# vlongle/pixie

Measured on AMD Instinct MI355X. Metric: voxels/s (128^3 U-Net fwd) + MPM particle-steps/s, higher is better.
Workload: dtype f32 (operands split fp16 hi+lo, 3 f16 MFMAs/product, fp32 accumulate); 1 GPU; 128^3x64 feature grid -> SegmentationUNet+RegressionUNet forward (+argmax/one-hot combine), 1 scene per GPU per step; grid=128, feature_channels=64, parallelism=scene-parallel x1, executor=c+hip_graph

## Files before the change

pixie_amd/csrc/conv3d_f16x3.hip:

```cpp
#include <hip/hip_runtime.h>

#include <cstdlib>
#include <map>
#include <string>
#include <type_traits>

#include "../../include/pixie_hip.h"
#include "common.h"
#include "conv_plan.h"

namespace pixie {

typedef float f32x16 __attribute__((ext_vector_type(16)));
typedef _Float16 f16x8 __attribute__((ext_vector_type(8)));

constexpr int kW16HeaderU4 = 4;

struct Conv16Args {
    const float* in0; const float* in1;
    int c0, cin;
    int ID, IH, IW;
    int LD, LH, LW;
    int ups;
    int stride;
    int OD, OH, OW;
    const float* pro_a; const float* pro_b; const float* gamma; const float* beta;
    int act;
    const uint4* w16;
    const float* wf;
    const float* bias;
    int cout, coutp;
    const float* residual; float* out;
    const unsigned* amax0; const unsigned* amax1;
    float in_bound;
    int TX, TY, TZ, lTX, lTY;
    int tiles_x, tiles_y, tiles_z, n_tiles;
    int HX, HY, HZ, HYX, CS;
    unsigned mHX, mHYX;
    float* stats; unsigned* out_amax;
    float* partial; int chunks_per_slice;
    int epi_lds;
    const float* sk_in0; const float* sk_in1;
    int sk_c0, sk_cin;
    const uint4* sk_w16; const float* sk_bias;
    const unsigned* sk_amax0; const unsigned* sk_amax1;
};

__device__ __forceinline__ int fast_div16(int n, int d, unsigned magic) {
    return (d == 1) ? n : (int)__umulhi((unsigned)n, magic);
}
__device__ __forceinline__ float act16(float t, int act) {
    if (act == 1) return t > 0.0f ? t : 0.02f * t;
    if (act == 2) return t / (1.0f + __expf(-t));
    return t;
}
__device__ __forceinline__ int scale_exponent(float bound) {
    const unsigned bits = __float_as_uint(bound);
    const int eb = (int)((bits >> 23) & 0xffu) - 127;
    if (!(bound > 0.0f) || eb > 100) return 0;
    int e = 14 - eb;
    return e > 100 ? 100 : (e < -100 ? -100 : e);
}
__device__ __forceinline__ float pow2i(int e) { return __uint_as_float((unsigned)(e + 127) << 23); }

template <int KS, int MB, int NB, bool EX = false, bool SP = false>
__device__ __forceinline__ void conv3d_f16x3_body(const Conv16Args& A) {
    static_assert(!SP || (KS == 3 && NB == 4 && !EX), "sub-pixel path: 3^3, two x parities x two voxel blocks per wave");
    extern __shared__ uint4 smem16[];
    constexpr int PAD = (KS == 3) ? 1 : 0;
    constexpr int NW = 4, NT = 64 * NW;
    const int bufsz = 4 * A.CS;

    const int tid = threadIdx.x;
    const int lane = tid & 63;
    const int wave = tid >> 6;
    const int kh = lane >> 5;
    const int l31 = lane & 31;

    int t = blockIdx.x;
    {
        const int per = (A.n_tiles + 7) >> 3;
        const int cand = (t & 7) * per + (t >> 3);
        if ((A.n_tiles & 7) == 0) t = cand;
    }
    int par = 0;
    if constexpr (SP) { par = t & 3; t >>= 2; }
    const int py = par & 1, pz = par >> 1;
    const int tx = t % A.tiles_x; t /= A.tiles_x;
    const int ty = t % A.tiles_y;
    const int tz = t / A.tiles_y;
    const int ox0 = tx * A.TX, oy0 = ty * A.TY, oz0 = tz * A.TZ;
    const int cout0 = blockIdx.y * (MB * 32);
    const int lx0 = SP ? ox0 - 1 : ox0 * A.stride - PAD;
    const int ly0 = SP ? oy0 - 1 + py : oy0 * A.stride - PAD;
    const int lz0 = SP ? oz0 - 1 + pz : oz0 * A.stride - PAD;
    const size_t ISP = (size_t)A.ID * A.IH * A.IW;
    const size_t OSP = (size_t)A.OD * A.OH * A.OW;

    int voff[NB];
    int ovox[NB];
    bool valid[NB];
#pragma unroll
    for (int nb = 0; nb < NB; ++nb) {
        if constexpr (SP) {
            const int px = nb >> 1;
            const int j = (wave * 2 + (nb & 1)) * 32 + l31;
            int x = j & (A.TX - 1);
            int y = (j >> A.lTX) & (A.TY - 1);
            int z = j >> (A.lTX + A.lTY);
            const int gx = 2 * (ox0 + x) + px, gy = 2 * (oy0 + y) + py, gz = 2 * (oz0 + z) + pz;
            const bool v = (z < A.TZ) && (gx < A.OW) && (gy < A.OH) && (gz < A.OD);
            if (!v) { x = 0; y = 0; z = 0; }
            voff[nb] = (z * A.HY + y) * A.HX + x + px + kh * A.CS;
            ovox[nb] = v ? (gz * A.OH + gy) * A.OW + gx : 0;
            valid[nb] = v;
            continue;
        }
        const int j = (wave * NB + nb) * 32 + l31;
        int x = j & (A.TX - 1);
        int y = (j >> A.lTX) & (A.TY - 1);
        int z = j >> (A.lTX + A.lTY);
        const bool v = (z < A.TZ) && (ox0 + x < A.OW) && (oy0 + y < A.OH) && (oz0 + z < A.OD);
        if (!v) { x = 0; y = 0; z = 0; }
        voff[nb] = ((z * A.HY + y) * A.HX + x) * A.stride + kh * A.CS;
        ovox[nb] = ((oz0 + z) * A.OH + (oy0 + y)) * A.OW + ox0 + x;
        valid[nb] = v;
    }

    float bound = A.in_bound;
    if (A.amax0) {
        bound = __uint_as_float(*A.amax0);
        if (A.amax1) bound = fmaxf(bound, __uint_as_float(*A.amax1));
    }
    const int ex = EX ? 0 : scale_exponent(bound);
    const float sx = pow2i(ex);

    f32x16 acc[MB][NB];
#pragma unroll
    for (int mb = 0; mb < MB; ++mb)
#pragma unroll
        for (int nb = 0; nb < NB; ++nb)
#pragma unroll
            for (int r = 0; r < 16; ++r) acc[mb][nb][r] = 0.0f;

    const int KG = A.cin >> 3;
    const size_t tap_stride = (size_t)KG * A.coutp;
    const size_t plane = (size_t)(SP ? 64 : KS * KS * KS) * tap_stride;
    const uint4* wHi = A.w16 + kW16HeaderU4 + (size_t)kh * A.coutp + cout0 + l31 + (size_t)(par * 16) * tap_stride;
    const uint4* wLo = wHi + plane;
    const float* wF = A.wf + (size_t)kh * A.coutp + cout0 + l31;
// ... 220 lines not shown
                        bl[s] = __builtin_bit_cast(f16x8, ldsLo[voff[px * 2 + s] + rowoff + ex]);
                    }
#pragma unroll
                    for (int mb = 0; mb < MB; ++mb)
#pragma unroll
                        for (int s = 0; s < 2; ++s)
                            acc[mb][px * 2 + s] = __builtin_amdgcn_mfma_f32_32x32x16_f16(al[mb], bh[s], acc[mb][px * 2 + s], 0, 0, 0);
#pragma unroll
                    for (int mb = 0; mb < MB; ++mb)
#pragma unroll
                        for (int s = 0; s < 2; ++s)
                            acc[mb][px * 2 + s] = __builtin_amdgcn_mfma_f32_32x32x16_f16(ah[mb], bl[s], acc[mb][px * 2 + s], 0, 0, 0);
#pragma unroll
                    for (int mb = 0; mb < MB; ++mb)
#pragma unroll
                        for (int s = 0; s < 2; ++s)
                            acc[mb][px * 2 + s] = __builtin_amdgcn_mfma_f32_32x32x16_f16(ah[mb], bh[s], acc[mb][px * 2 + s], 0, 0, 0);
#pragma unroll
                    for (int mb = 0; mb < MB; ++mb) { ah[mb] = ahn[mb]; al[mb] = aln[mb]; }
                }
            }
            __builtin_amdgcn_s_setprio(0);
            return;
        }
        f16x8 ah[MB], al[MB];
#pragma unroll
        for (int mb = 0; mb < MB; ++mb) {
            ah[mb] = __builtin_bit_cast(f16x8, wh[mb * 32]);
            al[mb] = __builtin_bit_cast(f16x8, wl[mb * 32]);
        }
#pragma unroll 1
        for (int zy = 0; zy < KS * KS; ++zy) {
            const int dz = zy / KS, dy = zy - dz * KS;
            const int rowoff = (dz * A.HY + dy) * A.HX;
#pragma unroll
            for (int dx = 0; dx < KS; ++dx) {
                const int tap = zy * KS + dx;
                const int nxt = (tap + 1 < TAPS) ? tap + 1 : tap;
                f16x8 ahn[MB], aln[MB];
#pragma unroll
                for (int mb = 0; mb < MB; ++mb) {
                    ahn[mb] = __builtin_bit_cast(f16x8, wh[(size_t)nxt * tap_stride + mb * 32]);
                    aln[mb] = __builtin_bit_cast(f16x8, wl[(size_t)nxt * tap_stride + mb * 32]);
                }
                __builtin_amdgcn_sched_barrier(0);
                f16x8 bh[NB], bl[NB];
#pragma unroll
                for (int nb = 0; nb < NB; ++nb) {
                    bh[nb] = __builtin_bit_cast(f16x8, ldsHi[voff[nb] + rowoff + dx]);
                    bl[nb] = __builtin_bit_cast(f16x8, ldsLo[voff[nb] + rowoff + dx]);
                }
#pragma unroll
                for (int mb = 0; mb < MB; ++mb)
#pragma unroll
                    for (int nb = 0; nb < NB; ++nb)
                        acc[mb][nb] = __builtin_amdgcn_mfma_f32_32x32x16_f16(al[mb], bh[nb], acc[mb][nb], 0, 0, 0);
#pragma unroll
                for (int mb = 0; mb < MB; ++mb)
#pragma unroll
                    for (int nb = 0; nb < NB; ++nb)
                        acc[mb][nb] = __builtin_amdgcn_mfma_f32_32x32x16_f16(ah[mb], bl[nb], acc[mb][nb], 0, 0, 0);
#pragma unroll
                for (int mb = 0; mb < MB; ++mb)
#pragma unroll
                    for (int nb = 0; nb < NB; ++nb)
                        acc[mb][nb] = __builtin_amdgcn_mfma_f32_32x32x16_f16(ah[mb], bh[nb], acc[mb][nb], 0, 0, 0);
#pragma unroll
                for (int mb = 0; mb < MB; ++mb) { ah[mb] = ahn[mb]; al[mb] = aln[mb]; }
            }
        }
        __builtin_amdgcn_s_setprio(0);
    };

    float inv2 = 0.0f;
    {
        const int c_begin = A.partial ? (int)blockIdx.z * A.chunks_per_slice * 16 : 0;
        const int c_end = A.partial ? min(A.cin, c_begin + A.chunks_per_slice * 16) : A.cin;
        for (int c_base = c_begin; c_base < c_end; c_base += 16) {
            __syncthreads();
            stage_chunk(c_base, smem16, tid, NT);
            __syncthreads();
            mfma_chunk(c_base, smem16);
        }
        if (!EX && !SP && A.sk_w16) {
            float sb = __uint_as_float(*A.sk_amax0);
            if (A.sk_amax1) sb = fmaxf(sb, __uint_as_float(*A.sk_amax1));
            const int ex2 = scale_exponent(sb);
            const float sx2 = pow2i(ex2);
            const float inv_main = __uint_as_float(A.w16[0].x) * pow2i(-ex);
            inv2 = __uint_as_float(A.sk_w16[0].x) * pow2i(-ex2);
            const float ratio = inv_main / inv2;
#pragma unroll
            for (int mb = 0; mb < MB; ++mb)
#pragma unroll
                for (int nb = 0; nb < NB; ++nb)
#pragma unroll
                    for (int r = 0; r < 16; ++r) acc[mb][nb][r] *= ratio;
            const int KG2 = A.sk_cin >> 3;
            const uint4* w2Hi = A.sk_w16 + kW16HeaderU4 + (size_t)kh * A.coutp + cout0 + l31;
            const uint4* w2Lo = w2Hi + (size_t)KG2 * A.coutp;
            const int centre = (KS == 3) ? (A.HY + 1) * A.HX + 1 : 0;
            const int tvox = A.TX * A.TY * A.TZ;
            for (int c2 = 0; c2 < A.sk_cin; c2 += 16) {
                f16x8 ah[MB], al[MB];
#pragma unroll
                for (int mb = 0; mb < MB; ++mb) {
                    ah[mb] = __builtin_bit_cast(f16x8, w2Hi[(size_t)(c2 >> 3) * A.coutp + mb * 32]);
                    al[mb] = __builtin_bit_cast(f16x8, w2Lo[(size_t)(c2 >> 3) * A.coutp + mb * 32]);
                }
                __syncthreads();
                uint4* bHi = smem16;
                uint4* bLo = smem16 + 2 * A.CS;
                for (int j = tid; j < tvox; j += NT) {
                    const int x = j & (A.TX - 1), y = (j >> A.lTX) & (A.TY - 1), z = j >> (A.lTX + A.lTY);
                    const bool okv = (ox0 + x < A.OW) && (oy0 + y < A.OH) && (oz0 + z < A.OD);
                    const size_t sidx = okv ? ((size_t)(oz0 + z) * A.IH + (oy0 + y)) * A.IW + ox0 + x : 0;
                    float val[16];
#pragma unroll
                    for (int q = 0; q < 16; ++q) {
                        const int cg = c2 + q;
                        const float* src = (cg < A.sk_c0) ? (A.sk_in0 + (size_t)cg * ISP) : (A.sk_in1 + (size_t)(cg - A.sk_c0) * ISP);
                        val[q] = src[sidx];
                    }
                    f16x8 vh[2], vl[2];
#pragma unroll
                    for (int q = 0; q < 16; ++q) {
                        const float sc = okv ? val[q] * sx2 : 0.0f;
                        const _Float16 hq = (_Float16)sc;
                        vh[q >> 3][q & 7] = hq;
                        vl[q >> 3][q & 7] = (_Float16)(sc - (float)hq);
                    }
                    const int slot = (z * A.HY + y) * A.HX + x + centre;
                    bHi[slot] = __builtin_bit_cast(uint4, vh[0]);
                    bHi[A.CS + slot] = __builtin_bit_cast(uint4, vh[1]);
                    bLo[slot] = __builtin_bit_cast(uint4, vl[0]);
                    bLo[A.CS + slot] = __builtin_bit_cast(uint4, vl[1]);
                }
                __syncthreads();
                f16x8 bh[NB], bl[NB];
#pragma unroll
                for (int nb = 0; nb < NB; ++nb) {
                    bh[nb] = __builtin_bit_cast(f16x8, bHi[voff[nb] + centre]);
                    bl[nb] = __builtin_bit_cast(f16x8, bLo[voff[nb] + centre]);
                }
#pragma unroll
                for (int mb = 0; mb < MB; ++mb)
#pragma unroll
                    for (int nb = 0; nb < NB; ++nb)
                        acc[mb][nb] = __builtin_amdgcn_mfma_f32_32x32x16_f16(al[mb], bh[nb], acc[mb][nb], 0, 0, 0);
#pragma unroll
                for (int mb = 0; mb < MB; ++mb)
#pragma unroll
                    for (int nb = 0; nb < NB; ++nb)
                        acc[mb][nb] = __builtin_amdgcn_mfma_f32_32x32x16_f16(ah[mb], bl[nb], acc[mb][nb], 0, 0, 0);
#pragma unroll
                for (int mb = 0; mb < MB; ++mb)
#pragma unroll
                    for (int nb = 0; nb < NB; ++nb)
                        acc[mb][nb] = __builtin_amdgcn_mfma_f32_32x32x16_f16(ah[mb], bh[nb], acc[mb][nb], 0, 0, 0);
            }
        }
    }

    const float inv = EX ? 1.0f : (A.sk_w16 ? inv2 : __uint_as_float(A.w16[0].x) * pow2i(-ex));
    if (A.partial) {
        float* dst = A.partial + (size_t)blockIdx.z * A.cout * OSP;
#pragma unroll
        for (int mb = 0; mb < MB; ++mb)
#pragma unroll
            for (int r = 0; r < 16; ++r) {
                const int co = cout0 + mb * 32 + (r & 3) + 8 * (r >> 2) + 4 * kh;
                if (co < A.cout) {
#pragma unroll
                    for (int nb = 0; nb < NB; ++nb)
                        if (valid[nb]) dst[(size_t)co * OSP + ovox[nb]] = acc[mb][nb][r] * inv;
                }
            }
        return;
    }
    float* red = reinterpret_cast<float*>(smem16);
    float wmax = 0.0f;
    const bool full = SP ? (A.epi_lds && cout0 + MB * 32 <= A.cout && (A.TX & 1) == 0 && (A.OW & 3) == 0 && NW * 64 <= A.TX * A.TY * A.TZ &&
                            2 * (ox0 + A.TX) <= A.OW && 2 * (oy0 + A.TY) <= A.OH && 2 * (oz0 + A.TZ) <= A.OD)
                         : (A.epi_lds && cout0 + MB * 32 <= A.cout && (A.TX & 3) == 0 && (A.OW & 3) == 0 && NW * NB * 32 <= A.TX * A.TY * A.TZ &&
                            ox0 + A.TX <= A.OW && oy0 + A.TY <= A.OH && oz0 + A.TZ <= A.OD);
    if (full) {
        constexpr int LDO = NB * 32 + 4;
        float* ldsO = reinterpret_cast<float*>(smem16) + wave * (32 * LDO);
        red = reinterpret_cast<float*>(smem16) + NW * 32 * LDO;
        constexpr int LPR = NB * 8;
        constexpr int RPI = 32 / LPR;
        constexpr int NIT = 16 / RPI;
        constexpr int G = 4;
        constexpr int GPB = NIT / G;
        constexpr int NGRP = MB * GPB;
        const int rsub = l31 / LPR, colq = 4 * (l31 % LPR), nbq = colq >> 5;
        const float* nobias = EX ? A.wf : reinterpret_cast<const float*>(A.w16);
        const bool hb0 = A.bias != nullptr, hb1 = A.sk_bias != nullptr;
        float braw[MB][2];
#pragma unroll
        for (int mb = 0; mb < MB; ++mb) {
            braw[mb][0] = (hb0 ? A.bias : nobias)[cout0 + mb * 32 + l31];
            braw[mb][1] = (hb1 ? A.sk_bias : nobias)[cout0 + mb * 32 + l31];
        }
        __syncthreads();
        const int jq = SP ? wave * 64 + (colq >> 1) : (wave * NB + nbq) * 32 + (colq & 31);
        const int xq = jq & (A.TX - 1), yq = (jq >> A.lTX) & (A.TY - 1), zq = jq >> (A.lTX + A.lTY);
        const size_t ovq = SP ? ((size_t)(2 * (oz0 + zq) + pz) * A.OH + (2 * (oy0 + yq) + py)) * A.OW + 2 * (ox0 + xq)
                              : ((size_t)(oz0 + zq) * A.OH + (oy0 + yq)) * A.OW + ox0 + xq;
        const size_t orow0 = (size_t)(cout0 + kh * RPI + rsub) * OSP + ovq;
        auto rows = [&](auto res_c, auto stats_c) {
            constexpr bool RES = decltype(res_c)::value, STATS = decltype(stats_c)::value;
            size_t step = (size_t)(2 * RPI) * OSP;
            asm volatile("" : "+s"(step));
            const float* pr = A.residual + orow0;
            float* po = A.out + orow0;
            float4 r4[2][G];
            auto fetch = [&](int q) {
#pragma unroll
                for (int g = 0; g < G; ++g) { r4[q & 1][g] = *reinterpret_cast<const float4*>(pr); pr += step; }
            };
#pragma unroll
            for (int q = 0; q < NGRP; ++q) {
                const int mb = q / GPB, it0 = (q % GPB) * G;
                asm volatile("" ::: "memory");
                if (q % GPB == 0) {
                    const int brow = __float_as_int((hb0 ? braw[mb][0] : 0.0f) + (hb1 ? braw[mb][1] : 0.0f));
#pragma unroll
                    for (int r = 0; r < 16; ++r) {
                        const int row = (r & 3) + 8 * (r >> 2);
                        const int blo = __builtin_amdgcn_readlane(brow, row), bhi = __builtin_amdgcn_readlane(brow, row + 4);
                        const float bv = __int_as_float(kh ? bhi : blo);
#pragma unroll
                        for (int nb = 0; nb < NB; ++nb)
                            ldsO[((r & 3) + 8 * (r >> 2) + 4 * kh) * LDO + (SP ? 2 * ((nb & 1) * 32 + l31) + (nb >> 1) : nb * 32 + l31)] =
                                __builtin_fmaf(acc[mb][nb][r], inv, bv);
                    }
                }
                if constexpr (RES) {
                    if (q == 0) fetch(0);
                    if (q + 1 < NGRP) fetch(q + 1);
                }
                float4 v4[G];
#pragma unroll
                for (int g = 0; g < G; ++g) {
                    const int rowl = (2 * (it0 + g) + kh) * RPI + rsub;
                    v4[g] = *reinterpret_cast<const float4*>(ldsO + rowl * LDO + colq);
                    if constexpr (RES) { v4[g].x += r4[q & 1][g].x; v4[g].y += r4[q & 1][g].y; v4[g].z += r4[q & 1][g].z; v4[g].w += r4[q & 1][g].w; }
                    *reinterpret_cast<float4*>(po) = v4[g]; po += step;
                }
                if constexpr (STATS) {
                    float s1[G], s2[G];
#pragma unroll
                    for (int g = 0; g < G; ++g) {
                        const float4 v = v4[g];
                        s1[g] = (v.x + v.y) + (v.z + v.w);
                        s2[g] = (v.x * v.x + v.y * v.y) + (v.z * v.z + v.w * v.w);
                        wmax = fmaxf(fmaxf(wmax, fmaxf(fabsf(v.x), fabsf(v.y))), fmaxf(fabsf(v.z), fabsf(v.w)));
                    }
                    asm volatile("" : "+v"(wmax));
#pragma unroll
                    for (int off = LPR / 2; off > 0; off >>= 1) {
                        float t1[G], t2[G];
#pragma unroll
                        for (int g = 0; g < G; ++g) { t1[g] = __shfl_xor(s1[g], off, 64); t2[g] = __shfl_xor(s2[g], off, 64); }
#pragma unroll
                        for (int g = 0; g < G; ++g) { s1[g] += t1[g]; s2[g] += t2[g]; }
                    }
                    if ((l31 % LPR) == 0) {
#pragma unroll
                        for (int g = 0; g < G; ++g) {
                            const int rowl = (2 * (it0 + g) + kh) * RPI + rsub;
                            red[(wave * MB * 32 + mb * 32 + rowl) * 2] = s1[g]; red[(wave * MB * 32 + mb * 32 + rowl) * 2 + 1] = s2[g];
                        }
                    }
                }
            }
        };
        using T = std::true_type; using F = std::false_type;
        if (A.residual) { if (A.stats) rows(T{}, T{}); else rows(T{}, F{}); }
        else { if (A.stats) rows(F{}, T{}); else rows(F{}, F{}); }
    } else {
    if (A.stats) __syncthreads();
#pragma unroll
    for (int mb = 0; mb < MB; ++mb) {
#pragma unroll
        for (int r = 0; r < 16; ++r) {
            const int row = mb * 32 + (r & 3) + 8 * (r >> 2) + 4 * kh;
            const int co = cout0 + row;
            float s1 = 0.0f, s2 = 0.0f;
            if (co < A.cout) {
                const float bv = (A.bias ? A.bias[co] : 0.0f) + (A.sk_bias ? A.sk_bias[co] : 0.0f);
#pragma unroll
                for (int nb = 0; nb < NB; ++nb) {
                    if (valid[nb]) {
                        const size_t o = (size_t)co * OSP + ovox[nb];
                        float val = acc[mb][nb][r] * inv + bv;
                        if (A.residual) val += A.residual[o];
                        A.out[o] = val;
                        s1 += val; s2 += val * val; wmax = fmaxf(wmax, fabsf(val));
                    }
                }
            }
            if (A.stats) {
#pragma unroll
                for (int off = 16; off > 0; off >>= 1) { s1 += __shfl_xor(s1, off, 64); s2 += __shfl_xor(s2, off, 64); }
                if (l31 == 0) { red[(wave * MB * 32 + row) * 2] = s1; red[(wave * MB * 32 + row) * 2 + 1] = s2; }
            }
        }
    }
    }
    if (A.stats) {
        __syncthreads();
        if (tid < MB * 32 * 2) {
            float t = red[tid];
#pragma unroll
            for (int w = 1; w < NW; ++w) t += red[w * MB * 64 + tid];
            A.stats[((size_t)blockIdx.x * A.coutp + cout0) * 2 + tid] = t;
        }
        if (A.out_amax) {
#pragma unroll
            for (int off = 32; off > 0; off >>= 1) wmax = fmaxf(wmax, __shfl_xor(wmax, off, 64));
            if (lane == 0 && wmax > 0.0f) atomicMax(A.out_amax, __float_as_uint(wmax));
        }
    }
}

template <int KS, int MB, int NB>
__global__ __launch_bounds__(256, 2) void conv3d_f16x3_kernel(Conv16Args A) {
    conv3d_f16x3_body<KS, MB, NB>(A);
}
template <int KS, int MB, int NB>
__global__ __launch_bounds__(256, 2) void conv3d_exact_kernel(Conv16Args A) {
    conv3d_f16x3_body<KS, MB, NB, true>(A);
}
template <int MB>
__global__ __launch_bounds__(256, 2) void conv3d_f16x3_subpixel_kernel(Conv16Args A) {
    conv3d_f16x3_body<3, MB, 4, false, true>(A);
}
__global__ __launch_bounds__(256, 2) void conv3d_f16x3_c64_fullres_kernel(Conv16Args A) {
    conv3d_f16x3_body<3, 2, 4>(A);
}

struct StatParts { const void* p; int n; long cstride, tstride; int f64; };

__device__ inline void block_channel_sums(const StatParts& P, int c, double* r, double& o1, double& o2) {
    double s1 = 0.0, s2 = 0.0;
    for (int t = threadIdx.x; t < P.n; t += 256) {
        const size_t k = ((size_t)c * P.cstride + (size_t)t * P.tstride) * 2;
        if (P.f64) { const double2 v = *reinterpret_cast<const double2*>(static_cast<const double*>(P.p) + k); s1 += v.x; s2 += v.y; }
        else { const float2 v = *reinterpret_cast<const float2*>(static_cast<const float*>(P.p) + k); s1 += v.x; s2 += v.y; }
    }
    for (int off = 32; off > 0; off >>= 1) { s1 += __shfl_down(s1, off, 64); s2 += __shfl_down(s2, off, 64); }
    if ((threadIdx.x & 63) == 0) { r[2 * (threadIdx.x >> 6)] = s1; r[2 * (threadIdx.x >> 6) + 1] = s2; }
    __syncthreads();
    o1 = r[0] + r[2] + r[4] + r[6]; o2 = r[1] + r[3] + r[5] + r[7];
    __syncthreads();
}

__global__ __launch_bounds__(256) void stats_finalize_kernel(StatParts P, double* __restrict__ sums) {
    const int c = blockIdx.x;
    __shared__ double r[8];
    double s1, s2;
    block_channel_sums(P, c, r, s1, s2);
    if (threadIdx.x == 0) { sums[2 * c] = s1; sums[2 * c + 1] = s2; }
}

__global__ __launch_bounds__(256) void stats_norm_finalize_kernel(StatParts P0, double* sums0, int c0, StatParts P1, double* sums1, int channels,
                                                                  double spatial, int mode, int groups, double eps,
                                                                  const float* __restrict__ weight, const float* __restrict__ bias,
                                                                  float* __restrict__ a, float* __restrict__ b) {
    __shared__ double r[8];
    const int cpg = mode == 0 ? 1 : channels / groups;
    const int first = blockIdx.x * cpg;
    double s1 = 0.0, s2 = 0.0;
    for (int k = first; k < first + cpg; ++k) {
        const bool in0 = k < c0;
        const StatParts& P = in0 ? P0 : P1;
        double* sums = in0 ? sums0 : sums1;
        const int kc = in0 ? k : k - c0;
        double t1, t2;
        if (P.n > 0) {
            block_channel_sums(P, kc, r, t1, t2);
            if (threadIdx.x == 0) { sums[2 * kc] = t1; sums[2 * kc + 1] = t2; }
        } else {
            t1 = sums[2 * kc]; t2 = sums[2 * kc + 1];
        }
        s1 += t1; s2 += t2;
    }
    const double cnt = mode == 0 ? spatial : spatial * cpg;
    const double mean = s1 / cnt;
    double var = s2 / cnt - mean * mean;
    if (var < 0.0) var = 0.0;
    const double rstd = 1.0 / sqrt(var + eps);
    for (int k = first + threadIdx.x; k < first + cpg; k += 256) {
        if (mode == 0) {
            a[k] = (float)rstd;
            b[k] = (float)(-mean * rstd);
        } else {
            const double w = weight ? (double)weight[k] : 1.0;
            const double bb = bias ? (double)bias[k] : 0.0;
            a[k] = (float)(rstd * w);
            b[k] = (float)(bb - mean * rstd * w);
        }
    }
}

__global__ __launch_bounds__(256) void splitk_reduce_kernel(const float* __restrict__ partial, int slices, long n_elems, long osp,
                                                            const float* __restrict__ bias, const float* residual, float* out) {
    const long i = (long)blockIdx.x * 256 + threadIdx.x;
    if (i >= n_elems) return;
    float v = partial[i];
    for (int s = 1; s < slices; ++s) v += partial[(size_t)s * n_elems + i];
// ... 198 lines not shown
    p.KS = s.ksize; p.coutp = pixie_conv_cout_padded(s.c_out);
    p.ups = s.upsample; p.LD = s.in_d << p.ups; p.LH = s.in_h << p.ups; p.LW = s.in_w << p.ups;
    const int cin = s.c0 + s.c1;
    const bool stride_ok = s.stride == 1 || (s.ksize == 3 && !s.upsample), chunks_ok = cin % 16 == 0;
    if (!s.w16) {
        if (!stride_ok || !chunks_ok || s.exact_v1) { p.path = CONV_FIRST_GEN; return p; }
        p.path = CONV_EXACT_TILED;
    } else {
        if (!stride_ok) return refuse(CONV_BAD_STRIDE);
        if (!chunks_ok || s.c0 % 8 != 0) return refuse(CONV_BAD_CHANNELS);
        if (s.subpixel && !(s.upsample == 1 && s.ksize == 3 && s.stride == 1 && !s.skip)) return refuse(CONV_BAD_SUBPIXEL);
        p.path = s.subpixel ? CONV_F16X3_SUBPIXEL : CONV_F16X3;
    }
    const bool sub = p.path == CONV_F16X3_SUBPIXEL;
    const int chunks = cin / 16;
    const int smax = (p.f16x3() && s.workspace) ? std::min(8, chunks / 2) : 1;
    auto tile = [&p](int ED, int EH, int EW, int vox) {
        p.TX = pow2_le(EW, 32);
        p.TY = pow2_le(EH, std::max(1, std::min(4, vox / p.TX)));
        p.TZ = std::max(1, std::min(ED, vox / (p.TX * p.TY)));
        p.lTX = ilog2(p.TX); p.lTY = ilog2(p.TY);
        p.tiles_x = (EW + p.TX - 1) / p.TX; p.tiles_y = (EH + p.TY - 1) / p.TY; p.tiles_z = (ED + p.TZ - 1) / p.TZ;
        p.n_tiles = p.tiles_x * p.tiles_y * p.tiles_z;
    };
    if (sub) {
        p.ups = 0; p.LD = s.in_d; p.LH = s.in_h; p.LW = s.in_w;
        tile((p.OD + 1) / 2, (p.OH + 1) / 2, (p.OW + 1) / 2, 256);
        p.n_tiles *= 4;
        p.HX = p.TX + 2; p.HY = p.TY + 1; p.HZ = p.TZ + 1;
        p.MB = (p.coutp >= 64) ? 2 : 1; p.NB = 4;
        const long wgs = (long)p.n_tiles * ((p.coutp + p.MB * 32 - 1) / (p.MB * 32));
        while (p.slices * 2 <= smax && wgs * p.slices < 512) p.slices *= 2;
    } else {
        const long ovol = (long)p.OD * p.OH * p.OW;
        int MB = (p.coutp >= 64) ? 2 : 1;
        int NB = (s.stride == 2) ? 1 : 4;
        auto n_wg = [&](int mb, int nb) {
            const long tiles = (ovol + 128L * nb - 1) / (128L * nb);
            return tiles * ((p.coutp + mb * 32 - 1) / (mb * 32));
        };
        int slices = 1;
        if (smax >= 2 && n_wg(MB, NB) < 512) {
            bool found = false;
            for (int nb = NB; nb >= 1 && !found; nb /= 2) {
                for (int sl = 1; sl <= smax; sl *= 2)
                    if (n_wg(MB, nb) * sl >= 512) { NB = nb; slices = sl; found = true; break; }
            }
            if (!found) { NB = 1; slices = 1; while (slices * 2 <= smax) slices *= 2; }
        } else {
            while (n_wg(MB, NB) < 512 && NB > 1) NB /= 2;
            if (n_wg(MB, NB) < 512 && MB > 1) MB = 1;
        }
        p.MB = MB; p.NB = NB; p.slices = slices;
        tile(p.OD, p.OH, p.OW, 128 * NB);
        p.HX = (p.TX - 1) * s.stride + s.ksize; p.HY = (p.TY - 1) * s.stride + s.ksize; p.HZ = (p.TZ - 1) * s.stride + s.ksize;
    }
    p.HYX = p.HY * p.HX; p.CS = p.HZ * p.HYX;
    p.mHX = magic_of(p.HX); p.mHYX = magic_of(p.HYX);
    if (p.slices > 1) p.chunks_per_slice = (chunks + p.slices - 1) / p.slices;
    p.lds_bytes = (size_t)4 * p.CS * sizeof(uint4);
    if (p.lds_bytes > 160 * 1024) return refuse(CONV_BAD_LDS);
    const size_t epi_bytes = ((size_t)4 * 32 * (p.NB * 32 + 4) + (size_t)4 * p.MB * 32 * 2) * sizeof(float);
    if (p.slices == 1 && epi_bytes <= 80 * 1024) { p.epi_lds = 1; p.lds_bytes = std::max(p.lds_bytes, epi_bytes); }
    p.grid = dim3((unsigned)p.n_tiles, (unsigned)((p.coutp + p.MB * 32 - 1) / (p.MB * 32)), (unsigned)p.slices);
    if (!p.f16x3()) return p;
    const long osp = (long)p.OD * p.OH * p.OW;
    if (p.slices > 1) {
        const int n = reduce_segments(osp);
        p.stats = ConvStatLayout{n, n, 1, 1};
        p.stats_floats = (int64_t)s.c_out * n * 2 * (int64_t)(sizeof(double) / sizeof(float));
        p.workspace_bytes = (int64_t)p.slices * s.c_out * osp * (int64_t)sizeof(float);
    } else {
        p.stats = ConvStatLayout{p.n_tiles, 1, p.coutp, 0};
        p.stats_floats = (int64_t)p.n_tiles * p.coutp * 2;
    }
    p.fullres = !sub && p.slices == 1 && s.ksize == 3 && p.MB == 2 && p.NB == 4 && cin == 64 && s.c_out == 64 && s.stride == 1 && !s.upsample &&
                s.c1 == 0 && !s.skip && osp >= 128L * 128 * 128;
    const int scin = s.skip_c0 + s.skip_c1;
    p.skip_foldable = !sub && s.stride == 1 && !s.upsample && scin > 0 && scin % 16 == 0 && s.skip_c0 % 8 == 0 && p.slices == 1;
    return p;
}

using ConvKernel = void (*)(Conv16Args);
static ConvKernel conv16_kernel(const ConvPlan& p) {
    if (p.path == CONV_F16X3_SUBPIXEL) return p.MB == 2 ? conv3d_f16x3_subpixel_kernel<2> : conv3d_f16x3_subpixel_kernel<1>;
    if (p.fullres) return conv3d_f16x3_c64_fullres_kernel;
#define PX_CONV16_PICK(KS_, MB_, NB_) \
    if (p.KS == KS_ && p.MB == MB_ && p.NB == NB_) return p.path == CONV_EXACT_TILED ? conv3d_exact_kernel<KS_, MB_, NB_> : conv3d_f16x3_kernel<KS_, MB_, NB_>;
    PX_CONV_VARIANTS(PX_CONV16_PICK)
#undef PX_CONV16_PICK
    return nullptr;
}

static int launch(ConvKernel kern, const ConvPlan& p, const Conv16Args& a, hipStream_t st) {
    PX_REQUIRE(kern != nullptr, "conv: no kernel variant for ksize=%d MB=%d NB=%d", p.KS, p.MB, p.NB);
    PX_CHECK_HIP(allow_max_dynamic_lds(reinterpret_cast<const void*>(kern)));
    hipLaunchKernelGGL(kern, p.grid, dim3(256), p.lds_bytes, st, a);
    PX_CHECK_HIP(hipGetLastError());
    return 0;
}

static Conv16Args conv16_args(const pixie_conv_desc* d, const ConvPlan& p) {
    Conv16Args a{};
    a.in0 = d->d_in0; a.in1 = d->d_in1; a.c0 = d->c0; a.cin = d->c0 + d->c1;
    a.ID = d->in_d; a.IH = d->in_h; a.IW = d->in_w;
    a.LD = p.LD; a.LH = p.LH; a.LW = p.LW; a.ups = p.ups; a.stride = d->stride;
    a.OD = p.OD; a.OH = p.OH; a.OW = p.OW;
    a.pro_a = d->d_pro_a; a.pro_b = d->d_pro_b; a.gamma = d->d_gamma; a.beta = d->d_beta; a.act = d->act;
    a.bias = d->d_bias; a.cout = d->c_out; a.coutp = p.coutp;
    a.residual = d->d_residual; a.out = d->d_out;
    a.TX = p.TX; a.TY = p.TY; a.TZ = p.TZ; a.lTX = p.lTX; a.lTY = p.lTY;
    a.tiles_x = p.tiles_x; a.tiles_y = p.tiles_y; a.tiles_z = p.tiles_z; a.n_tiles = p.n_tiles;
    a.HX = p.HX; a.HY = p.HY; a.HZ = p.HZ; a.HYX = p.HYX; a.CS = p.CS; a.mHX = p.mHX; a.mHYX = p.mHYX;
    a.chunks_per_slice = p.chunks_per_slice; a.epi_lds = p.epi_lds;
    return a;
}

int conv3d_f16x3_forward(const pixie_conv_desc* d, const ConvPlan& p, hipStream_t st) {
    PX_REQUIRE(p.refusal != CONV_BAD_STRIDE, "f16x3 conv: stride must be 1, or 2 for a 3^3 kernel");
    PX_REQUIRE(p.refusal != CONV_BAD_CHANNELS, "f16x3 conv: c_in must be a multiple of 16 (got %d+%d)", d->c0, d->c1);
    PX_REQUIRE(d->d_in_amax0 != nullptr || d->in_bound > 0.0f, "f16x3 conv: needs d_in_amax0 or a positive in_bound");
    PX_REQUIRE(d->c1 == 0 || d->d_in_amax0 == nullptr || d->d_in_amax1 != nullptr, "f16x3 conv: second input needs its own amax slot");
    PX_REQUIRE(p.refusal != CONV_BAD_SUBPIXEL, "f16x3 conv: sub-pixel weights need upsample = 1, ksize = 3, stride = 1 and no folded skip");
    Conv16Args a = conv16_args(d, p);
    a.w16 = reinterpret_cast<const uint4*>(d->d_w16);
    a.amax0 = d->d_in_amax0; a.amax1 = (d->c1 > 0) ? d->d_in_amax1 : nullptr; a.in_bound = d->in_bound;
    a.stats = d->d_out_stats; a.out_amax = d->d_out_amax;
    if (d->d_skip_w16) {
        PX_REQUIRE(p.skip_foldable, "f16x3 conv: this launch cannot fold a skip convolution (pixie_conv_skip_foldable)");
        PX_REQUIRE(d->d_skip_in0 && d->d_skip_amax0 && (d->skip_c1 == 0 || (d->d_skip_in1 && d->d_skip_amax1)), "f16x3 conv: folded skip needs its inputs and their amax slots");
        a.sk_in0 = d->d_skip_in0; a.sk_in1 = d->d_skip_in1; a.sk_c0 = d->skip_c0; a.sk_cin = d->skip_c0 + d->skip_c1;
        a.sk_w16 = reinterpret_cast<const uint4*>(d->d_skip_w16); a.sk_bias = d->d_skip_bias;
        a.sk_amax0 = d->d_skip_amax0; a.sk_amax1 = d->skip_c1 > 0 ? d->d_skip_amax1 : nullptr;
    }
    if (p.slices > 1) {
        a.partial = static_cast<float*>(d->d_workspace);
        a.stats = nullptr; a.out_amax = nullptr;
    }
    PX_REQUIRE(p.refusal != CONV_BAD_LDS, "f16x3 conv: tile needs %zu B of LDS", p.lds_bytes);
    PX_REQUIRE(p.f16x3(), "f16x3 conv: bad sizes");
    if (int rc = launch(conv16_kernel(p), p, a, st)) return rc;
    if (p.slices == 1) return 0;
    const long osp = (long)a.OD * a.OH * a.OW, n_elems = (long)a.cout * osp;
    if (d->d_out_stats) {
        const dim3 rgrid((unsigned)reduce_segments(osp), (unsigned)a.cout);
        double* rstats = reinterpret_cast<double*>(d->d_out_stats);
        PX_REQUIRE((reinterpret_cast<size_t>(rstats) & 7) == 0, "f16x3 conv: d_out_stats of a split-K launch must be 8-byte aligned");
        const bool vec = osp % 4 == 0 && ((reinterpret_cast<size_t>(a.partial) | reinterpret_cast<size_t>(a.residual) | reinterpret_cast<size_t>(a.out)) & 15) == 0;
        if (vec) hipLaunchKernelGGL(splitk_reduce_stats_kernel<true>, rgrid, dim3(256), 0, st, a.partial, p.slices, n_elems, osp, a.bias, a.residual,
                                    a.out, rstats, d->d_out_amax);
        else hipLaunchKernelGGL(splitk_reduce_stats_kernel<false>, rgrid, dim3(256), 0, st, a.partial, p.slices, n_elems, osp, a.bias, a.residual,
                                a.out, rstats, d->d_out_amax);
    } else {
        hipLaunchKernelGGL(splitk_reduce_kernel, dim3((unsigned)((n_elems + 255) / 256)), dim3(256), 0, st, a.partial, p.slices, n_elems, osp,
                           a.bias, a.residual, a.out);
    }
    PX_CHECK_HIP(hipGetLastError());
    return 0;
}

int conv3d_exact_forward(const pixie_conv_desc* d, const ConvPlan& p, hipStream_t st) {
    PX_REQUIRE(p.refusal != CONV_BAD_LDS, "exact conv: tile needs %zu B of LDS", p.lds_bytes);
    PX_REQUIRE(p.path == CONV_EXACT_TILED, "exact conv: bad sizes");
    Conv16Args a = conv16_args(d, p);
    a.wf = d->d_w;
    a.in_bound = 1.0f;
    return launch(conv16_kernel(p), p, a, st);
}

}

using namespace pixie;

static ConvPlan plan_of(const pixie_conv_desc* d) { return d ? conv_plan(conv_shape_of(d)) : ConvPlan{}; }
static StatParts stat_parts(const ConvPlan& p, const void* stats) { return StatParts{stats, p.stats.n, p.stats.cstride, p.stats.tstride, p.stats.f64}; }

extern "C" int64_t pixie_conv_stats_floats(const pixie_conv_desc* d) { return plan_of(d).stats_floats; }

extern "C" int64_t pixie_conv_workspace_bytes(const pixie_conv_desc* d) {
    if (!d) return 0;
    ConvShape s = conv_shape_of(d);
    s.workspace = true;
    return conv_plan(s).workspace_bytes;
}

#ifdef PIXIE_DIAG
extern "C" int pixie_conv_kernel_variant(const pixie_conv_desc* d, int* slices_out) {
    const ConvPlan p = plan_of(d);
    if (slices_out) *slices_out = p.f16x3() ? p.slices : 1;
    if (!p.f16x3()) return 0;
    if (p.path == CONV_F16X3_SUBPIXEL) return 8300 + p.MB * 10 + p.NB;
    if (p.fullres) return 9324;
    return p.KS * 100 + p.MB * 10 + p.NB;
}

extern "C" int pixie_conv_tile_geometry(const pixie_conv_desc* d, int32_t out[10]) {
    const ConvPlan p = plan_of(d);
    if (!out || !p.tiled()) return 1;
    const int32_t v[10] = {p.TX, p.TY, p.TZ, p.tiles_x, p.tiles_y, p.tiles_z, p.epi_lds, p.slices, p.MB, p.NB};
    for (int i = 0; i < 10; ++i) out[i] = v[i];
    return 0;
}

extern "C" int pixie_conv_stats_layout(const pixie_conv_desc* d, int64_t out[6]) {
    const ConvPlan p = plan_of(d);
    if (!out || !p.f16x3()) return 1;
    out[0] = p.stats.n; out[1] = p.stats.cstride; out[2] = p.stats.tstride; out[3] = p.stats.f64; out[4] = p.stats.f64 ? kReduceSeg : 0;
    out[5] = p.coutp;
    return 0;
}
#endif

extern "C" int pixie_conv_skip_foldable(const pixie_conv_desc* d) { return plan_of(d).skip_foldable ? 1 : 0; }

extern "C" int pixie_stats_finalize(const float* d_stats, const pixie_conv_desc* d, double* d_sums, void* stream) {
    PX_REQUIRE(d_stats && d && d_sums, "pixie_stats_finalize: null argument");
    hipLaunchKernelGGL(stats_finalize_kernel, dim3((unsigned)d->c_out), dim3(256), 0, as_stream(stream), stat_parts(plan_of(d), d_stats), d_sums);
    PX_CHECK_HIP(hipGetLastError());
    return 0;
}

extern "C" int pixie_stats_norm_finalize(const float* d_stats0, const pixie_conv_desc* desc0, double* d_sums0, const float* d_stats1,
                                         const pixie_conv_desc* desc1, double* d_sums1, int c1, int64_t spatial, int mode, int groups,
                                         double eps, const float* d_weight, const float* d_bias, float* d_a, float* d_b, void* stream) {
// ... 67 lines not shown
```

Measured before the change: 25.25 million voxels/s.

## Feed folded skip convolution from registers via buffer loads instead of LDS staging

Splits the folded-skip path into a separate kernel template. When the skip channel split is 16-aligned, each lane loads its own voxels' skip-input channels directly with raw buffer loads, converts them to hi/lo f16 in registers, and issues the MFMAs without the LDS round-trip and the two block barriers per chunk. The LDS-staged path is kept for misaligned channel splits, and the plain kernel no longer carries the skip code at all, which may lower register pressure. The cost is uncoalesced-ish per-lane channel-strided global loads, plus a new 4 GiB limit on the span of the skip input.

Measured after the change: 25.56 million voxels/s, median of 6. 1.2% higher.

```diff
diff --git a/pixie_amd/csrc/conv3d_f16x3.hip b/pixie_amd/csrc/conv3d_f16x3.hip
--- a/pixie_amd/csrc/conv3d_f16x3.hip
+++ b/pixie_amd/csrc/conv3d_f16x3.hip
@@ -63,9 +63,10 @@
 }
 __device__ __forceinline__ float pow2i(int e) { return __uint_as_float((unsigned)(e + 127) << 23); }
 
-template <int KS, int MB, int NB, bool EX = false, bool SP = false>
+template <int KS, int MB, int NB, bool EX = false, bool SP = false, int SK = 0>
 __device__ __forceinline__ void conv3d_f16x3_body(const Conv16Args& A) {
     static_assert(!SP || (KS == 3 && NB == 4 && !EX), "sub-pixel path: 3^3, two x parities x two voxel blocks per wave");
+    static_assert(SK == 0 || (!EX && !SP), "folded skip (SK: 1 register-fed, 2 staged through LDS): f16x3, no sub-pixel form");
     extern __shared__ uint4 smem16[];
     constexpr int PAD = (KS == 3) ? 1 : 0;
     constexpr int NW = 4, NT = 64 * NW;
@@ -452,7 +453,7 @@
             __syncthreads();
             mfma_chunk(c_base, smem16);
         }
-        if (!EX && !SP && A.sk_w16) {
+        if constexpr (SK != 0) {
             float sb = __uint_as_float(*A.sk_amax0);
             if (A.sk_amax1) sb = fmaxf(sb, __uint_as_float(*A.sk_amax1));
             const int ex2 = scale_exponent(sb);
@@ -466,73 +467,137 @@
                 for (int nb = 0; nb < NB; ++nb)
 #pragma unroll
                     for (int r = 0; r < 16; ++r) acc[mb][nb][r] *= ratio;
-            const int KG2 = A.sk_cin >> 3;
-            const uint4* w2Hi = A.sk_w16 + kW16HeaderU4 + (size_t)kh * A.coutp + cout0 + l31;
-            const uint4* w2Lo = w2Hi + (size_t)KG2 * A.coutp;
-            const int centre = (KS == 3) ? (A.HY + 1) * A.HX + 1 : 0;
-            const int tvox = A.TX * A.TY * A.TZ;
-            for (int c2 = 0; c2 < A.sk_cin; c2 += 16) {
-                f16x8 ah[MB], al[MB];
-#pragma unroll
-                for (int mb = 0; mb < MB; ++mb) {
-                    ah[mb] = __builtin_bit_cast(f16x8, w2Hi[(size_t)(c2 >> 3) * A.coutp + mb * 32]);
-                    al[mb] = __builtin_bit_cast(f16x8, w2Lo[(size_t)(c2 >> 3) * A.coutp + mb * 32]);
-                }
-                __syncthreads();
-                uint4* bHi = smem16;
-                uint4* bLo = smem16 + 2 * A.CS;
-                for (int j = tid; j < tvox; j += NT) {
+            auto sk_chunks = [&]() {
+                int l31s = l31, khs = kh, waves = wave;
+                asm volatile("" : "+v"(l31s), "+v"(khs), "+v"(waves));
+                const unsigned chb = 4u * (unsigned)ISP;
+                unsigned off[NB];
+#pragma unroll
+                for (int nb = 0; nb < NB; ++nb) {
+                    const int j = (waves * NB + nb) * 32 + l31s;
                     const int x = j & (A.TX - 1), y = (j >> A.lTX) & (A.TY - 1), z = j >> (A.lTX + A.lTY);
-                    const bool okv = (ox0 + x < A.OW) && (oy0 + y < A.OH) && (oz0 + z < A.OD);
-                    const size_t sidx = okv ? ((size_t)(oz0 + z) * A.IH + (oy0 + y)) * A.IW + ox0 + x : 0;
-                    float val[16];
-#pragma unroll
-                    for (int q = 0; q < 16; ++q) {
-                        const int cg = c2 + q;
-                        const float* src = (cg < A.sk_c0) ? (A.sk_in0 + (size_t)cg * ISP) : (A.sk_in1 + (size_t)(cg - A.sk_c0) * ISP);
-                        val[q] = src[sidx];
+                    off[nb] = (valid[nb] ? 4u * (unsigned)(((oz0 + z) * A.IH + (oy0 + y)) * A.IW + ox0 + x) : 0u) + 8u * (unsigned)khs * chb;
+                }
+                const unsigned wlane = 16u * (unsigned)(khs * A.coutp + l31s);
+                const char* w2Hi = reinterpret_cast<const char*>(A.sk_w16 + kW16HeaderU4 + cout0);
+                const char* w2Lo = w2Hi + (size_t)(A.sk_cin >> 3) * A.coutp * sizeof(uint4);
+#pragma unroll 1
+                for (int c2 = 0; c2 < A.sk_cin; c2 += 16) {
+                    f16x8 ah[MB], al[MB];
+                    const size_t wrow = (size_t)(c2 >> 3) * A.coutp * sizeof(uint4);
+#pragma unroll
+                    for (int mb = 0; mb < MB; ++mb) {
+                        al[mb] = __builtin_bit_cast(f16x8, *reinterpret_cast<const uint4*>(w2Lo + wrow + mb * 32 * sizeof(uint4) + wlane));
+                        ah[mb] = __builtin_bit_cast(f16x8, *reinterpret_cast<const uint4*>(w2Hi + wrow + mb * 32 * sizeof(uint4) + wlane));
                     }
-                    f16x8 vh[2], vl[2];
-#pragma unroll
-                    for (int q = 0; q < 16; ++q) {
-                        const float sc = okv ? val[q] * sx2 : 0.0f;
-                        const _Float16 hq = (_Float16)sc;
-                        vh[q >> 3][q & 7] = hq;
-                        vl[q >> 3][q & 7] = (_Float16)(sc - (float)hq);
+                    const float* base = (c2 < A.sk_c0) ? (A.sk_in0 + (size_t)c2 * ISP) : (A.sk_in1 + (size_t)(c2 - A.sk_c0) * ISP);
+                    const __amdgpu_buffer_rsrc_t rsrc = __builtin_amdgcn_make_buffer_rsrc(const_cast<float*>(base), 0, -1, 0x00020000);
+                    float v[NB][8];
+#pragma unroll
+                    for (int q = 0; q < 8; ++q)
+#pragma unroll
+                        for (int nb = 0; nb < NB; ++nb)
+                            v[nb][q] = __uint_as_float(__builtin_amdgcn_raw_buffer_load_b32(rsrc, (int)off[nb], (int)((unsigned)q * chb), 0));
+                    __builtin_amdgcn_sched_barrier(0);
+                    f16x8 bh[NB], bl[NB];
+#pragma unroll
+                    for (int nb = 0; nb < NB; ++nb)
+#pragma unroll
+                        for (int q = 0; q < 8; ++q) {
+                            const float sc = valid[nb] ? v[nb][q] * sx2 : 0.0f;
+                            const _Float16 hq = (_Float16)sc;
+                            bh[nb][q] = hq;
+                            bl[nb][q] = (_Float16)(sc - (float)hq);
+                        }
+#pragma unroll
+                    for (int mb = 0; mb < MB; ++mb)
+#pragma unroll
+                        for (int nb = 0; nb < NB; ++nb)
+                            acc[mb][nb] = __builtin_amdgcn_mfma_f32_32x32x16_f16(al[mb], bh[nb], acc[mb][nb], 0, 0, 0);
+#pragma unroll
+                    for (int mb = 0; mb < MB; ++mb)
+#pragma unroll
+                        for (int nb = 0; nb < NB; ++nb)
+                            acc[mb][nb] = __builtin_amdgcn_mfma_f32_32x32x16_f16(ah[mb], bl[nb], acc[mb][nb], 0, 0, 0);
+#pragma unroll
+                    for (int mb = 0; mb < MB; ++mb)
+#pragma unroll
+                        for (int nb = 0; nb < NB; ++nb)
+                            acc[mb][nb] = __builtin_amdgcn_mfma_f32_32x32x16_f16(ah[mb], bh[nb], acc[mb][nb], 0, 0, 0);
+                    __builtin_amdgcn_sched_barrier(0);
+                }
+            };
+            if constexpr (SK == 2) {
+                const int KG2 = A.sk_cin >> 3;
+                const uint4* w2Hi = A.sk_w16 + kW16HeaderU4 + (size_t)kh * A.coutp + cout0 + l31;
+                const uint4* w2Lo = w2Hi + (size_t)KG2 * A.coutp;
+                const int centre = (KS == 3) ? (A.HY + 1) * A.HX + 1 : 0;
+                const int tvox = A.TX * A.TY * A.TZ;
+                for (int c2 = 0; c2 < A.sk_cin; c2 += 16) {
+                    f16x8 ah[MB], al[MB];
+#pragma unroll
+                    for (int mb = 0; mb < MB; ++mb) {
+                        ah[mb] = __builtin_bit_cast(f16x8, w2Hi[(size_t)(c2 >> 3) * A.coutp + mb * 32]);
+                        al[mb] = __builtin_bit_cast(f16x8, w2Lo[(size_t)(c2 >> 3) * A.coutp + mb * 32]);
                     }
-                    const int slot = (z * A.HY + y) * A.HX + x + centre;
-                    bHi[slot] = __builtin_bit_cast(uint4, vh[0]);
-                    bHi[A.CS + slot] = __builtin_bit_cast(uint4, vh[1]);
-                    bLo[slot] = __builtin_bit_cast(uint4, vl[0]);
-                    bLo[A.CS + slot] = __builtin_bit_cast(uint4, vl[1]);
-                }
-                __syncthreads();
-                f16x8 bh[NB], bl[NB];
-#pragma unroll
-                for (int nb = 0; nb < NB; ++nb) {
-                    bh[nb] = __builtin_bit_cast(f16x8, bHi[voff[nb] + centre]);
-                    bl[nb] = __builtin_bit_cast(f16x8, bLo[voff[nb] + centre]);
-                }
-#pragma unroll
-                for (int mb = 0; mb < MB; ++mb)
-#pragma unroll
-                    for (int nb = 0; nb < NB; ++nb)
-                        acc[mb][nb] = __builtin_amdgcn_mfma_f32_32x32x16_f16(al[mb], bh[nb], acc[mb][nb], 0, 0, 0);
-#pragma unroll
-                for (int mb = 0; mb < MB; ++mb)
-#pragma unroll
-                    for (int nb = 0; nb < NB; ++nb)
-                        acc[mb][nb] = __builtin_amdgcn_mfma_f32_32x32x16_f16(ah[mb], bl[nb], acc[mb][nb], 0, 0, 0);
-#pragma unroll
-                for (int mb = 0; mb < MB; ++mb)
-#pragma unroll
-                    for (int nb = 0; nb < NB; ++nb)
-                        acc[mb][nb] = __builtin_amdgcn_mfma_f32_32x32x16_f16(ah[mb], bh[nb], acc[mb][nb], 0, 0, 0);
-            }
-        }
-    }
-
-    const float inv = EX ? 1.0f : (A.sk_w16 ? inv2 : __uint_as_float(A.w16[0].x) * pow2i(-ex));
+                    __syncthreads();
+                    uint4* bHi = smem16;
+                    uint4* bLo = smem16 + 2 * A.CS;
+                    for (int j = tid; j < tvox; j += NT) {
+                        const int x = j & (A.TX - 1), y = (j >> A.lTX) & (A.TY - 1), z = j >> (A.lTX + A.lTY);
+                        const bool okv = (ox0 + x < A.OW) && (oy0 + y < A.OH) && (oz0 + z < A.OD);
+                        const size_t sidx = okv ? ((size_t)(oz0 + z) * A.IH + (oy0 + y)) * A.IW + ox0 + x : 0;
+                        float val[16];
+#pragma unroll
+                        for (int q = 0; q < 16; ++q) {
+                            const int cg = c2 + q;
+                            const float* src = (cg < A.sk_c0) ? (A.sk_in0 + (size_t)cg * ISP) : (A.sk_in1 + (size_t)(cg - A.sk_c0) * ISP);
+                            val[q] = src[sidx];
+                        }
+                        f16x8 vh[2], vl[2];
+#pragma unroll
+                        for (int q = 0; q < 16; ++q) {
+                            const float sc = okv ? val[q] * sx2 : 0.0f;
+                            const _Float16 hq = (_Float16)sc;
+                            vh[q >> 3][q & 7] = hq;
+                            vl[q >> 3][q & 7] = (_Float16)(sc - (float)hq);
+                        }
+                        const int slot = (z * A.HY + y) * A.HX + x + centre;
+                        bHi[slot] = __builtin_bit_cast(uint4, vh[0]);
+                        bHi[A.CS + slot] = __builtin_bit_cast(uint4, vh[1]);
+                        bLo[slot] = __builtin_bit_cast(uint4, vl[0]);
+                        bLo[A.CS + slot] = __builtin_bit_cast(uint4, vl[1]);
+                    }
+                    __syncthreads();
+                    f16x8 bh[NB], bl[NB];
+#pragma unroll
+                    for (int nb = 0; nb < NB; ++nb) {
+                        bh[nb] = __builtin_bit_cast(f16x8, bHi[voff[nb] + centre]);
+                        bl[nb] = __builtin_bit_cast(f16x8, bLo[voff[nb] + centre]);
+                    }
+#pragma unroll
+                    for (int mb = 0; mb < MB; ++mb)
+#pragma unroll
+                        for (int nb = 0; nb < NB; ++nb)
+                            acc[mb][nb] = __builtin_amdgcn_mfma_f32_32x32x16_f16(al[mb], bh[nb], acc[mb][nb], 0, 0, 0);
+#pragma unroll
+                    for (int mb = 0; mb < MB; ++mb)
+#pragma unroll
+                        for (int nb = 0; nb < NB; ++nb)
+                            acc[mb][nb] = __builtin_amdgcn_mfma_f32_32x32x16_f16(ah[mb], bl[nb], acc[mb][nb], 0, 0, 0);
+#pragma unroll
+                    for (int mb = 0; mb < MB; ++mb)
+#pragma unroll
+                        for (int nb = 0; nb < NB; ++nb)
+                            acc[mb][nb] = __builtin_amdgcn_mfma_f32_32x32x16_f16(ah[mb], bh[nb], acc[mb][nb], 0, 0, 0);
+                }
+            } else {
+                sk_chunks();
+            }
+        }
+    }
+
+    const float inv = EX ? 1.0f : (SK != 0 ? inv2 : __uint_as_float(A.w16[0].x) * pow2i(-ex));
     if (A.partial) {
         float* dst = A.partial + (size_t)blockIdx.z * A.cout * OSP;
 #pragma unroll
@@ -699,6 +764,10 @@
 template <int KS, int MB, int NB>
 __global__ __launch_bounds__(256, 2) void conv3d_f16x3_kernel(Conv16Args A) {
     conv3d_f16x3_body<KS, MB, NB>(A);
+}
+template <int KS, int MB, int NB, bool STAGED>
+__global__ __launch_bounds__(256, 2) void conv3d_f16x3_skip_kernel(Conv16Args A) {
+    conv3d_f16x3_body<KS, MB, NB, false, false, STAGED ? 2 : 1>(A);
 }
 template <int KS, int MB, int NB>
 __global__ __launch_bounds__(256, 2) void conv3d_exact_kernel(Conv16Args A) {
@@ -1063,11 +1132,14 @@
 }
 
 using ConvKernel = void (*)(Conv16Args);
-static ConvKernel conv16_kernel(const ConvPlan& p) {
+static ConvKernel conv16_kernel(const ConvPlan& p, bool skip = false, int skip_c0 = 0) {
     if (p.path == CONV_F16X3_SUBPIXEL) return p.MB == 2 ? conv3d_f16x3_subpixel_kernel<2> : conv3d_f16x3_subpixel_kernel<1>;
     if (p.fullres) return conv3d_f16x3_c64_fullres_kernel;
-#define PX_CONV16_PICK(KS_, MB_, NB_) \
-    if (p.KS == KS_ && p.MB == MB_ && p.NB == NB_) return p.path == CONV_EXACT_TILED ? conv3d_exact_kernel<KS_, MB_, NB_> : conv3d_f16x3_kernel<KS_, MB_, NB_>;
+#define PX_CONV16_PICK(KS_, MB_, NB_)                                                                \
+    if (p.KS == KS_ && p.MB == MB_ && p.NB == NB_)                                                   \
+        return p.path == CONV_EXACT_TILED ? conv3d_exact_kernel<KS_, MB_, NB_>                       \
+                                          : (!skip ? conv3d_f16x3_kernel<KS_, MB_, NB_>                                \
+                                                   : ((skip_c0 & 8) ? conv3d_f16x3_skip_kernel<KS_, MB_, NB_, true> : conv3d_f16x3_skip_kernel<KS_, MB_, NB_, false>));
     PX_CONV_VARIANTS(PX_CONV16_PICK)
 #undef PX_CONV16_PICK
     return nullptr;
@@ -1110,6 +1182,7 @@
     if (d->d_skip_w16) {
         PX_REQUIRE(p.skip_foldable, "f16x3 conv: this launch cannot fold a skip convolution (pixie_conv_skip_foldable)");
         PX_REQUIRE(d->d_skip_in0 && d->d_skip_amax0 && (d->skip_c1 == 0 || (d->d_skip_in1 && d->d_skip_amax1)), "f16x3 conv: folded skip needs its inputs and their amax slots");
+        PX_REQUIRE((int64_t)d->in_d * d->in_h * d->in_w * 16 * (int64_t)sizeof(float) < (int64_t)1 << 32, "f16x3 conv: folded skip: 16 channels of the skip input must span less than 4 GiB");
         a.sk_in0 = d->d_skip_in0; a.sk_in1 = d->d_skip_in1; a.sk_c0 = d->skip_c0; a.sk_cin = d->skip_c0 + d->skip_c1;
         a.sk_w16 = reinterpret_cast<const uint4*>(d->d_skip_w16); a.sk_bias = d->d_skip_bias;
         a.sk_amax0 = d->d_skip_amax0; a.sk_amax1 = d->skip_c1 > 0 ? d->d_skip_amax1 : nullptr;
@@ -1120,7 +1193,7 @@
     }
     PX_REQUIRE(p.refusal != CONV_BAD_LDS, "f16x3 conv: tile needs %zu B of LDS", p.lds_bytes);
     PX_REQUIRE(p.f16x3(), "f16x3 conv: bad sizes");
-    if (int rc = launch(conv16_kernel(p), p, a, st)) return rc;
+    if (int rc = launch(conv16_kernel(p, a.sk_w16 != nullptr, a.sk_c0), p, a, st)) return rc;
     if (p.slices == 1) return 0;
     const long osp = (long)a.OD * a.OH * a.OW, n_elems = (long)a.cout * osp;
     if (d->d_out_stats) {
```
